# andreeaiana/newsreclib

Measured on AMD Instinct MI355X. Metric: impressions/sec (train step) NRMS MINDsmall-shape, higher is better.
Workload: dtype f32 (projections: 3xbf16 split MFMA); 1 GPU; NRMS pretrained-emb (d=300, 15 heads, Q=200) MINDsmall-shaped train step: B=128/GPU, H=50, C=5, L=30, V=70000, dropout 0.2, Adam lr 1e-4 (BASELINE.json configs[1]); global_batch=128, parallelism=dp1, gemm_engine=bf16x3

## Files before the change

### include/newsreclib_amd.h

```cpp
#ifndef NEWSRECLIB_AMD_H
#define NEWSRECLIB_AMD_H

#include <stddef.h>
#include <stdint.h>

#ifdef __cplusplus
extern "C" {
#endif

#define NRL_ABI_VERSION 19

#define NRL_OK 0
#define NRL_E_INVALID (-1)
#define NRL_E_WORKSPACE (-2)
#define NRL_E_HIP (-3)

typedef struct NrlBlockParams {
  const float* in_proj_weight;
  const float* in_proj_bias;
  const float* out_proj_weight;
  const float* out_proj_bias;
  const float* att_weight;
  const float* att_bias;
  const float* att_query;
// ... 26 lines not shown
int32_t nrl_get_options(void);

int nrl_prof_enable(int32_t on);
int nrl_prof_read(double* total_ms, int64_t* launches, double* total_flops);

uint32_t nrl_dropout_key(uint64_t seed, uint32_t stream);
int nrl_dropout_mask(uint8_t* keep, int64_t n_elems, double p, uint64_t seed, uint32_t stream,
                     void* stream_handle);

size_t nrl_sort_positions_workspace_bytes(int64_t n, int64_t vocab);
int nrl_sort_positions(const int64_t* ids, int64_t n, int64_t vocab, int64_t* order, void* ws, size_t ws_bytes,
                       void* stream);

size_t nrl_news_encoder_workspace_bytes(int64_t n_news, int32_t seq_len, int32_t embed_dim,
                                        int32_t num_heads, int32_t query_dim);
int nrl_news_encoder_fwd(const NrlBlockParams* p, const float* emb_table, int64_t vocab,
                         const int64_t* ids, int64_t n_news, int32_t seq_len, double p_drop,
                         uint64_t seed, uint32_t stream0, int32_t save_for_backward, float* out,
                         void* ws, size_t ws_bytes, void* stream);
int32_t nrl_token_table_supported(int32_t seq_len, int32_t embed_dim, int32_t num_heads, int32_t query_dim);
size_t nrl_token_table_bytes(int64_t vocab, int32_t embed_dim, int32_t num_heads, int32_t query_dim);
int nrl_token_table_build(const NrlBlockParams* p, const float* emb_table, int64_t vocab, void* table, size_t table_bytes,
                          void* stream);
size_t nrl_news_encoder_fwd_table_workspace_bytes(int64_t n_news, int32_t seq_len, int32_t num_heads);
int nrl_news_encoder_fwd_table(const NrlBlockParams* p, const void* table, size_t table_bytes, int64_t vocab,
                               const int64_t* ids, int64_t n_news, int32_t seq_len, float* out, void* ws, size_t ws_bytes,
                               void* stream);
int nrl_news_encoder_bwd(const NrlBlockParams* p, const NrlBlockGrads* g, const float* emb_table,
                         float* d_emb_table, int64_t vocab, const int64_t* ids, const int64_t* sorted_positions,
                         int64_t n_news, int32_t seq_len, double p_drop, uint64_t seed,
// ... 192 lines not shown
                            void* ws, size_t ws_bytes, int32_t image_ready, void* stream);
int nrl_linear_dgrad_gelu_img(const float* w, const float* d_c, const float* pre, int64_t m, int32_t n, int32_t k, float* d_pre,
                              void* ws, size_t ws_bytes, int32_t image_ready, void* stream);
int32_t nrl_linear_gelu_supported(int32_t n_wide);
int32_t nrl_linear3_supported(int32_t n, int32_t k);
size_t nrl_linear3_workspace_bytes(int32_t n, int32_t k);
int nrl_linear3_fwd_img(const float* a, const float* w0, const float* w1, const float* w2, const float* b0, const float* b1,
                        const float* b2, int64_t m, int32_t n, int32_t k, float* c, void* ws, size_t ws_bytes, int32_t image_ready,
                        void* stream);
int nrl_linear3_dgrad_img(const float* d_c, const float* w0, const float* w1, const float* w2, int64_t m, int32_t n, int32_t k,
                          const float* add, float* d_a, void* ws, size_t ws_bytes, int32_t image_ready, void* stream);
int nrl_linear_dgrad_add_img(const float* d_c, const float* w, int64_t m, int32_t n, int32_t k, const float* add, float* d_a,
                             void* ws, size_t ws_bytes, int32_t image_ready, void* stream);
int nrl_embedding_grad(const float* d_out, const int64_t* ids, const int64_t* sorted_positions, int64_t n_ids, int32_t dim,
                       int64_t padding_idx, float* d_table, void* stream);
size_t nrl_linear_workspace_bytes(int32_t n, int32_t k);
int nrl_linear_fwd(const float* a, const float* w, const float* bias, int64_t m, int32_t n,
                   int32_t k, float* c, void* ws, size_t ws_bytes, void* stream);
int nrl_linear_bwd(const float* a, const float* w, const float* d_c, int64_t m, int32_t n, int32_t k, float* d_a,
                   float* d_w, float* d_bias, void* ws, size_t ws_bytes, void* stream);
int nrl_linear_fwd_img(const float* a, const float* w, const float* bias, int64_t m, int32_t n, int32_t k,
                       float* c, void* ws, size_t ws_bytes, int32_t image_ready, void* stream);
int nrl_linear_bwd_img(const float* a, const float* w, const float* d_c, int64_t m, int32_t n, int32_t k, float* d_a,
                       float* d_w, float* d_bias, void* ws, size_t ws_bytes, int32_t image_ready, void* stream);

int32_t nrl_sdpa_supported(int64_t n_batch, int32_t seq_len, int32_t num_heads, int32_t head_dim);
int nrl_sdpa_fwd(const float* q, const float* k, const float* v, const uint8_t* key_keep, int64_t n_batch, int32_t seq_len,
                 int32_t num_heads, int32_t head_dim, float scale, double p_drop, uint64_t seed, uint32_t stream0, float* out,
                 float* lse, void* stream);
int nrl_sdpa_bwd(const float* q, const float* k, const float* v, const uint8_t* key_keep, const float* out, const float* d_out,
// ... 252 lines not shown
```

### newsreclib_amd/_lib.py

```python
from __future__ import annotations

import ctypes
import os
from ctypes import POINTER, c_char_p, c_double, c_float, c_int32, c_int64, c_size_t, c_uint8, c_uint32, c_uint64, c_void_p

_PKG = os.path.dirname(os.path.abspath(__file__))
LIB_PATH = os.path.join(_PKG, "libnewsreclib_amd.so")
ABI_VERSION = 19


class NrlBlockParams(ctypes.Structure):
    _fields_ = [
        ("in_proj_weight", c_void_p), ("in_proj_bias", c_void_p),
        ("out_proj_weight", c_void_p), ("out_proj_bias", c_void_p),
        ("att_weight", c_void_p), ("att_bias", c_void_p), ("att_query", c_void_p),
        ("embed_dim", c_int32), ("num_heads", c_int32), ("query_dim", c_int32), ("gemm_engine", c_int32),
        ("options", c_int32),
    ]


OPTIONS_EXPLICIT = 0x40000000


class NrlBlockGrads(ctypes.Structure):
# ... 87 lines not shown
SIGNATURES = {
    "nrl_abi_version": (c_int32, []),
    "nrl_build_id": (c_char_p, []),
    "nrl_last_error": (c_char_p, []),
    "nrl_set_gemm_engine": (c_int32, [c_int32]),
    "nrl_get_gemm_engine": (c_int32, []),
    "nrl_set_option": (c_int32, [c_char_p, c_int32]),
    "nrl_get_options": (c_int32, []),
    "nrl_prof_enable": (c_int32, [c_int32]),
    "nrl_prof_read": (c_int32, [POINTER(c_double), POINTER(c_int64), POINTER(c_double)]),
    "nrl_dropout_key": (c_uint32, [c_uint64, c_uint32]),
    "nrl_dropout_mask": (c_int32, [c_void_p, c_int64, c_double, c_uint64, c_uint32, c_void_p]),
    "nrl_sort_positions_workspace_bytes": (c_size_t, [c_int64, c_int64]),
    "nrl_sort_positions": (c_int32, [c_void_p, c_int64, c_int64, c_void_p, c_void_p, c_size_t, c_void_p]),
    "nrl_news_encoder_workspace_bytes": (c_size_t, [c_int64, c_int32, c_int32, c_int32, c_int32]),
    "nrl_news_encoder_fwd": (c_int32, [POINTER(NrlBlockParams), c_void_p, c_int64, c_void_p, c_int64, c_int32,
                                       c_double, c_uint64, c_uint32, c_int32, c_void_p, c_void_p, c_size_t,
                                       c_void_p]),
    "nrl_token_table_supported": (c_int32, [c_int32, c_int32, c_int32, c_int32]),
    "nrl_token_table_bytes": (c_size_t, [c_int64, c_int32, c_int32, c_int32]),
    "nrl_token_table_build": (c_int32, [POINTER(NrlBlockParams), c_void_p, c_int64, c_void_p, c_size_t, c_void_p]),
    "nrl_news_encoder_fwd_table_workspace_bytes": (c_size_t, [c_int64, c_int32, c_int32]),
    "nrl_news_encoder_fwd_table": (c_int32, [POINTER(NrlBlockParams), c_void_p, c_size_t, c_int64, c_void_p, c_int64, c_int32,
                                             c_void_p, c_void_p, c_size_t, c_void_p]),
    "nrl_news_encoder_bwd": (c_int32, [POINTER(NrlBlockParams), POINTER(NrlBlockGrads), c_void_p, c_void_p, c_int64,
                                       c_void_p, c_void_p, c_int64, c_int32, c_double, c_uint64, c_uint32,
                                       c_void_p, c_int32, c_void_p, c_size_t, c_void_p]),
    "nrl_user_encoder_workspace_bytes": (c_size_t, [c_int64, c_int64, c_int32, c_int32, c_int32]),
    "nrl_user_encoder_fwd": (c_int32, [POINTER(NrlBlockParams), c_void_p, c_int64, c_int64, c_double, c_uint64,
                                       c_uint32, c_int32, c_int32, c_void_p, c_void_p, c_size_t, c_void_p]),
# ... 189 lines not shown
                                     c_size_t, c_int32, c_void_p]),
    "nrl_linear_gelu_fwd_img": (c_int32, [c_void_p, c_void_p, c_void_p, c_int64, c_int32, c_int32, c_void_p, c_void_p, c_void_p,
                                          c_size_t, c_int32, c_void_p]),
    "nrl_linear_dgrad_gelu_img": (c_int32, [c_void_p, c_void_p, c_void_p, c_int64, c_int32, c_int32, c_void_p, c_void_p, c_size_t,
                                            c_int32, c_void_p]),
    "nrl_linear_gelu_supported": (c_int32, [c_int32]),
    "nrl_linear3_supported": (c_int32, [c_int32, c_int32]),
    "nrl_linear3_workspace_bytes": (c_size_t, [c_int32, c_int32]),
    "nrl_linear3_fwd_img": (c_int32, [c_void_p, c_void_p, c_void_p, c_void_p, c_void_p, c_void_p, c_void_p, c_int64, c_int32, c_int32,
                                      c_void_p, c_void_p, c_size_t, c_int32, c_void_p]),
    "nrl_linear3_dgrad_img": (c_int32, [c_void_p, c_void_p, c_void_p, c_void_p, c_int64, c_int32, c_int32, c_void_p, c_void_p,
                                        c_void_p, c_size_t, c_int32, c_void_p]),
    "nrl_linear_dgrad_add_img": (c_int32, [c_void_p, c_void_p, c_int64, c_int32, c_int32, c_void_p, c_void_p, c_void_p, c_size_t,
                                           c_int32, c_void_p]),
    "nrl_embedding_grad": (c_int32, [c_void_p, c_void_p, c_void_p, c_int64, c_int32, c_int64, c_void_p, c_void_p]),
    "nrl_linear_bwd_img": (c_int32, [c_void_p, c_void_p, c_void_p, c_int64, c_int32, c_int32, c_void_p, c_void_p, c_void_p,
                                     c_void_p, c_size_t, c_int32, c_void_p]),
}

_lib = None


def load() -> ctypes.CDLL:
    global _lib
    if _lib is not None:
        return _lib
    import torch
    if not os.path.exists(LIB_PATH):
        raise RuntimeError(
            f"{LIB_PATH} is missing: the HIP extension was not built (run `python -m newsreclib_amd._build` "
# ... 22 lines not shown


def set_gemm_engine(name: str) -> None:
    if name not in ENGINES:
        raise ValueError(f"unknown GEMM engine {name!r}; choose from {sorted(ENGINES)}")
    check(load().nrl_set_gemm_engine(ENGINES[name]), "nrl_set_gemm_engine")


def get_gemm_engine() -> str:
    code = load().nrl_get_gemm_engine()
    return {v: k for k, v in ENGINES.items()}[code]


OPTION_NAMES = ("news_fused", "news_fused_bwd", "news_attn_mfma", "news_planes", "news_od_planes", "news_aa_planes",
                "wgrad_2step", "wgrad_ws", "rowpanel", "x3_dma", "news_tail", "news_tail_bwd", "user_fork", "news_fork",
                "news_qkv_planes", "news_pad_share", "news_tail_od", "user_proj")


def set_option(name: str, value: bool) -> None:
    check(load().nrl_set_option(name.encode(), int(bool(value))), "nrl_set_option")


def options_mask() -> int:
    return int(load().nrl_get_options())


def options_word() -> int:
    return OPTIONS_EXPLICIT | options_mask()


def require_options(mask: int, what: str) -> None:
# ... 20 lines not shown
```

### newsreclib_amd/csrc/nrl_api.hip

```cpp
#include "nrl_api_internal.h"

namespace nrl {

static thread_local char g_err[512] = "";

void set_error(const char* fmt, ...) {
  va_list ap;
  va_start(ap, fmt);
  vsnprintf(g_err, sizeof(g_err), fmt, ap);
  va_end(ap);
}

ProfState g_prof;
std::atomic<int> g_default_engine{ENGINE_BF16X3};
thread_local int t_engine = -1;
thread_local int64_t t_opts = -1;

static const char* const kOptName[O_COUNT] = {"news_fused", "news_fused_bwd", "news_attn_mfma", "news_planes", "news_od_planes",
                                              "news_aa_planes", "wgrad_2step", "wgrad_ws", "rowpanel", "x3_dma", "news_tail",
                                              "news_tail_bwd", "user_fork", "news_fork", "news_qkv_planes", "news_pad_share", "news_tail_od", "user_proj"};
static const char* const kOptEnv[O_COUNT] = {"NRL_NEWS_FUSED", "NRL_NEWS_FUSED_BWD", "NRL_NEWS_ATTN_MFMA", "NRL_NEWS_PLANES",
                                             "NRL_NEWS_OD_PLANES", "NRL_NEWS_AA_PLANES", "NRL_WGRAD_2STEP", "NRL_WGRAD_WS",
                                             "NRL_ROWPANEL", "NRL_X3_DMA", "NRL_NEWS_TAIL", "NRL_NEWS_TAIL_BWD", "NRL_USER_FORK",
                                             "NRL_NEWS_FORK", "NRL_NEWS_QKV_PLANES", "NRL_NEWS_PAD_SHARE", "NRL_NEWS_TAIL_OD", "NRL_USER_PROJ"};
std::atomic<uint32_t> g_opt_default{[] {
  uint32_t m = 0;
  for (int i = 0; i < O_COUNT; ++i) {
    const bool dflt = i != O_NEWS_FUSED_BWD && i != O_USER_FORK && i != O_NEWS_TAIL_OD;
    const char* e = getenv(kOptEnv[i]);
    bool v = e == nullptr ? dflt : (dflt ? e[0] != '0' : e[0] == '1');
    if (opt_retired(i)) v = false;
    m |= v ? (1u << i) : 0u;
  }
  return m;
}()};

struct ForkSet {
  hipStream_t s[2] = {nullptr, nullptr};
  hipEvent_t fork = nullptr, join[2] = {nullptr, nullptr};
};
static int fork_set(ForkSet** out) {
  thread_local ForkSet sets[64];
  int dev = 0;
  NRL_HIP(hipGetDevice(&dev));
  ForkSet& f = sets[dev & 63];
  if (f.fork == nullptr) {
    for (int i = 0; i < 2; ++i) {
      NRL_HIP(hipStreamCreateWithFlags(&f.s[i], hipStreamNonBlocking));
      NRL_HIP(hipEventCreateWithFlags(&f.join[i], hipEventDisableTiming));
    }
    NRL_HIP(hipEventCreateWithFlags(&f.fork, hipEventDisableTiming));
  }
  *out = &f;
  return NRL_OK;
}

constexpr int LIN_PANEL_BLOCKS = 16;
static inline int lin_panels(int n_out) { return (n_out + 16 * LIN_PANEL_BLOCKS - 1) / (16 * LIN_PANEL_BLOCKS); }
static inline size_t lin_image_elems(int n_out, int k_red) {
  return (size_t)lin_panels(n_out) * rp_image_elems(LIN_PANEL_BLOCKS, rp_kblocks(k_red, false));
}
static inline bool lin_panels_on(int n_out) { return opt(O_ROWPANEL) && n_out >= 16 * LIN_PANEL_BLOCKS; }
template <class Epi>
static int linear_panels(const float* a, const float* src, int64_t sn, int64_t sk, int n_out, int k_red, const Epi& epi,
                         int64_t m, uint16_t* img, hipStream_t st, bool build = true) {
// ... 53 lines not shown
}
int nrl_get_gemm_engine(void) { return g_default_engine.load(); }

int nrl_set_option(const char* name, int32_t value) {
  NRL_REQUIRE(name != nullptr, "set_option: null name");
  for (int i = 0; i < O_COUNT; ++i)
    if (!strcmp(name, kOptName[i])) {
      NRL_REQUIRE(value == 0 || !opt_retired(i), "set_option: '%s' was retired in ABI v14 (its kernel lost its A/B and lives in "
                  "tools/experimental/; the bit is reserved and must stay 0)", name);
      if (value != 0) g_opt_default.fetch_or(1u << i);
      else g_opt_default.fetch_and(~(1u << i));
      return NRL_OK;
    }
  set_error("set_option: unknown option '%s' (news_fused, news_fused_bwd, news_attn_mfma, news_planes, news_od_planes, "
            "news_aa_planes, wgrad_2step, wgrad_ws, rowpanel, x3_dma, news_tail, news_tail_bwd, user_fork, news_fork, news_qkv_planes, "
            "news_pad_share, news_tail_od, user_proj)", name);
  return NRL_E_INVALID;
}

int32_t nrl_get_options(void) { return (int32_t)g_opt_default.load(); }

uint32_t nrl_dropout_key(uint64_t seed, uint32_t stream) { return dropout_key(seed, stream); }

int nrl_dropout_mask(uint8_t* keep, int64_t n_elems, double p, uint64_t seed, uint32_t stream,
                     void* stream_handle) {
  NRL_REQUIRE(keep != nullptr && n_elems >= 0 && p >= 0.0 && p < 1.0, "dropout_mask: bad arguments");
  return dropout_mask(keep, n_elems, make_dropout(p, seed, stream), (hipStream_t)stream_handle);
}

size_t nrl_news_encoder_workspace_bytes(int64_t n_news, int32_t seq_len, int32_t embed_dim,
                                        int32_t num_heads, int32_t query_dim) {
// ... 210 lines not shown
  NRL_TRY(block_planes(p, s, w, false, &bp, st, slabs ? s.heads : 0));
  sb_.forked = news_fork_on(sb_);
  SideFork side;
  hipEvent_t side_in_join = nullptr;
  if (phase != 2) {
    if (sb_.forked) {
      ForkSet* fs = nullptr;
      NRL_TRY(fork_set(&fs));
      side.s = fs->s[0]; side.fork = fs->fork; side.join = fs->join[0];
    }
    NRL_TRY(block_bwd_phase1(p, g, sb_, w, bp, d2, d_out, st, slabs, sb_.forked ? &side : nullptr));
    if (slabs) {
      NewsAttnBwdArgs a;
      a.qkv_hm = w.qkv; a.d_o = w.d_o; a.lse = w.lse; a.dqkv = w.dqkv; a.n_news = n_news; a.L = seq_len; a.D = s.D;
      a.heads = s.heads; a.scale = s.geom.scale; a.hpw = 1; a.planes = planes ? 1 : 0;
      if (planes && opt(O_NEWS_QKV_PLANES)) NRL_TRY(launch_news_attn_bwd_p(a, st));
      else NRL_TRY(launch_news_attn_bwd(a, st));
      if (news_fork_in_on(sb_, planes)) {
        ForkSet* fs = nullptr;
        NRL_TRY(fork_set(&fs));
        const int si = news_fork_in_mode() == 2 ? 0 : 1;
        NRL_HIP(hipEventRecord(fs->fork, st));
        NRL_HIP(hipStreamWaitEvent(fs->s[si], fs->fork, 0));
        NRL_TRY(block_wgrad_in_planes(g, w.x, sb_, w, fs->s[si]));
        NRL_HIP(hipEventRecord(fs->join[1], fs->s[si]));
        side_in_join = fs->join[1];
      }
    }
    const KCSlab dq_hp{w.dqkv, s.M};
    const KCPlanes dq_pl{reinterpret_cast<const unsigned char*>(w.dqkv), s.pad_rows};
    if (sorted_positions != nullptr) {
      float* dx = w.d_o;
      const EpiLinear epi{dx, s.D, nullptr, 0, d1, s.D};
// ... 9 lines not shown
        if (planes) NRL_TRY(rp_dispatch(dq_pl, bp.rp.in_d_hp, EpiNewsRows<EpiLinear>{epi, seq_len}, s.pad_rows, s.D, s.heads * 64, st));
        else if (slabs) NRL_TRY(rp_dispatch(dq_hp, bp.rp.in_d_hp, epi, s.M, s.D, s.heads * 64, st));
        else NRL_TRY(gemm_dgrad(w.dqkv, p->in_proj_weight, bp.in, epi, s.M, 3 * s.D, s.D, st, bp.rp.on ? &bp.rp.in_d : nullptr));
        NRL_TRY(embedding_grad_sorted(dx, ids, sorted_positions, s.M, s.D, d_emb_table, st));
      }
    } else {
      const EpiScatter epi{d_emb_table, ids, s.D, d1};
      if (planes) NRL_TRY(rp_dispatch(dq_pl, bp.rp.in_d_hp, EpiNewsRows<EpiScatter>{epi, seq_len}, s.pad_rows, s.D, s.heads * 64, st));
      else if (slabs) NRL_TRY(rp_dispatch(dq_hp, bp.rp.in_d_hp, epi, s.M, s.D, s.heads * 64, st));
      else NRL_TRY(gemm_dgrad(w.dqkv, p->in_proj_weight, bp.in, epi, s.M, 3 * s.D, s.D, st, bp.rp.on ? &bp.rp.in_d : nullptr));
    }
  }
  if (phase != 2 && sb_.forked) NRL_HIP(hipStreamWaitEvent(st, side.join, 0));
  if (side_in_join != nullptr) NRL_HIP(hipStreamWaitEvent(st, side_in_join, 0));
  if (phase != 1) NRL_TRY(block_bwd_phase2(g, w.x, sb_, w, st, slabs, planes));
  return NRL_OK;
}

size_t nrl_user_encoder_workspace_bytes(int64_t batch, int64_t hist_len, int32_t embed_dim,
                                        int32_t num_heads, int32_t query_dim) {
  return block_ws_floats(batch * hist_len, embed_dim, query_dim, num_heads, true) * sizeof(float);
}

int nrl_user_encoder_fwd(const NrlBlockParams* p, const float* hist, int64_t batch, int64_t hist_len,
                         double p_drop, uint64_t seed, uint32_t stream0, int32_t input_dropout,
                         int32_t save_for_backward, float* out, void* ws, size_t ws_bytes, void* stream) {
  NRL_TRY(check_params(p));
  const EngineScope engine_scope(p->gemm_engine);
  const OptScope opt_scope(p->options);
  NRL_REQUIRE(hist && out && batch > 0 && hist_len > 0, "user_encoder_fwd: bad arguments");
// ... 231 lines not shown
  return launch_rp_gemm<LIN_PANEL_BLOCKS, 4, 0, 2>(A, im, EpiStore{d_a, k}, m, k, 3 * n, st, P);
}

int nrl_linear_dgrad_add_img(const float* d_c, const float* w, int64_t m, int32_t n, int32_t k, const float* add, float* d_a,
                             void* ws, size_t ws_bytes, int32_t image_ready, void* stream) {
  NRL_REQUIRE(d_c && w && add && d_a && m >= 0 && n > 0 && k > 0 && k % 4 == 0 && n % 4 == 0, "linear_dgrad_add: bad arguments");
  NRL_REQUIRE((((uintptr_t)d_c | (uintptr_t)w | (uintptr_t)add | (uintptr_t)d_a) & 15) == 0, "linear_dgrad_add: 16-byte alignment");
  NRL_REQUIRE(cur_engine() == ENGINE_BF16X3 && lin_panels_on(k), "linear_dgrad_add: bf16x3 engine and k >= 256 (nrl_linear_gelu_supported)");
  NRL_REQUIRE(ws != nullptr && ((uintptr_t)ws & 255) == 0 && ws_bytes >= nrl_linear_workspace_bytes(n, k), "linear_dgrad_add: workspace");
  if (m == 0) return NRL_OK;
  return linear_panels(d_c, w, 1, k, k, n, EpiAddStore{d_a, k, add}, m, (uint16_t*)ws, (hipStream_t)stream, image_ready == 0);
}

int32_t nrl_linear_gelu_supported(int32_t n_wide) { return (cur_engine() == ENGINE_BF16X3 && lin_panels_on(n_wide)) ? 1 : 0; }

int nrl_embedding_grad(const float* d_out, const int64_t* ids, const int64_t* sorted_positions, int64_t n_ids, int32_t dim,
                       int64_t padding_idx, float* d_table, void* stream) {
  NRL_REQUIRE(d_out && ids && sorted_positions && d_table && n_ids >= 0 && dim > 0, "embedding_grad: bad arguments");
  return embedding_grad_any(d_out, ids, sorted_positions, n_ids, dim, padding_idx, d_table, (hipStream_t)stream);
}

size_t nrl_linear_workspace_bytes(int32_t n, int32_t k) {
  size_t e = split_weight_elems(n, k);
  if (lin_image_elems(n, k) > e) e = lin_image_elems(n, k);
  if (lin_image_elems(k, n) > e) e = lin_image_elems(k, n);
  return align_up(e * sizeof(uint16_t), 256);
}

int nrl_linear_fwd(const float* a, const float* w, const float* bias, int64_t m, int32_t n, int32_t k,
                   float* c, void* ws, size_t ws_bytes, void* stream) {
// ... 61 lines not shown
```

### newsreclib_amd/csrc/nrl_api_internal.h

```cpp
#pragma once
#include <stdarg.h>
#include <stdlib.h>
#include <string.h>

#include <atomic>
#include <utility>
#include <vector>

#include "nrl_gemm.h"
#include "nrl_gemm_bf16x3.h"
#include "nrl_gemm_bf16x3_dma.h"
#include "nrl_rowpanel.h"
#include "nrl_gemm_ws.h"
#include "nrl_news_fused.h"
#include "nrl_news_tail_api.h"
#include "nrl_user_tail.h"
#include "nrl_wgrad_planes.h"
#include "nrl_kernels.h"
#include "nrl_conv.h"
#include "nrl_gru_fused.h"

namespace nrl {

struct ProfState {
// ... 41 lines not shown

enum { ENGINE_F32 = 0, ENGINE_BF16X3 = 1 };
extern std::atomic<int> g_default_engine;
extern thread_local int t_engine;
static inline int cur_engine() { return t_engine >= 0 ? t_engine : g_default_engine.load(std::memory_order_relaxed); }
struct EngineScope {
  int prev;
  explicit EngineScope(int per_call) : prev(t_engine) {
    t_engine = per_call > 0 ? per_call - 1 : g_default_engine.load(std::memory_order_relaxed);
  }
  ~EngineScope() { t_engine = prev; }
};
static inline bool engine_field_ok(int v) { return v >= 0 && v <= 2; }
enum {
  O_NEWS_FUSED = 0, O_NEWS_FUSED_BWD, O_NEWS_ATTN_MFMA, O_NEWS_PLANES, O_NEWS_OD_PLANES, O_NEWS_AA_PLANES, O_WGRAD_2STEP,
  O_WGRAD_WS, O_ROWPANEL, O_X3_DMA, O_NEWS_TAIL, O_NEWS_TAIL_BWD, O_USER_FORK, O_NEWS_FORK, O_NEWS_QKV_PLANES, O_NEWS_PAD_SHARE, O_NEWS_TAIL_OD, O_USER_PROJ, O_COUNT
};
static inline bool opt_retired(int bit) { return bit == O_NEWS_FUSED_BWD || bit == O_NEWS_TAIL_OD; }
extern std::atomic<uint32_t> g_opt_default;
extern thread_local int64_t t_opts;
static inline bool opt(int bit) {
  const uint32_t m = t_opts >= 0 ? (uint32_t)t_opts : g_opt_default.load(std::memory_order_relaxed);
  return (m >> bit) & 1u;
}
struct OptScope {
  int64_t prev;
  explicit OptScope(int32_t per_call) : prev(t_opts) {
    t_opts = (per_call & NRL_OPTIONS_EXPLICIT) ? (int64_t)(per_call & ((1 << O_COUNT) - 1))
                                               : (int64_t)g_opt_default.load(std::memory_order_relaxed);
  }
  ~OptScope() { t_opts = prev; }
// ... 538 lines not shown
  }
  if (!attention_elsewhere) {
    if (block_attn_x3(s)) NRL_TRY(attn_bwd_x3(w.qkv, w.o, w.d_o, w.lse, w.dqkv, s.geom, st));
    else NRL_TRY(attn_bwd(w.qkv, w.o, w.d_o, w.lse, w.dqkv, s.geom, st));
  }
  return NRL_OK;
}

static inline int news_fork_in_mode() {
  static const int v = [] { const char* e = getenv("NRL_NEWS_FORK_IN"); return e != nullptr ? atoi(e) : 2; }();
  return v;
}
static inline bool news_fork_in_on(const BlockShape& s, bool bf16_planes) {
  return news_fork_in_mode() != 0 && bf16_planes && news_fork_on(s) && s.forked;
}
static int block_wgrad_in_planes(const NrlBlockGrads* G, const float* x_rows, const BlockShape& s, const BlockWs& w, hipStream_t st) {
  const int D = s.D;
  const size_t scratch_avail = opt(O_WGRAD_2STEP) ? qkv_elems(s.M, s.D, s.heads, s.pad_rows) : 0;
  static const int wp_splits = [] { const char* e = getenv("NRL_WGRAD_PLANES_SPLITS"); return e ? atoi(e) : 32; }();
  const EpiAtomicWBHeads epi_w{G->in_proj_weight, D, G->in_proj_bias, D, s.heads, s.dh};
  float* const sc_w = wgrad_planes_scratch_floats(s.heads, 20, wp_splits) <= scratch_avail ? w.qkv : nullptr;
  if (wgrad_planes_waves() == 4) return launch_wgrad_planes<0, 4>(w.dqkv, x_rows, s.pool_groups, s.heads, 20, D + 1, epi_w, wp_splits, st, sc_w);
  return launch_wgrad_planes<0, 8>(w.dqkv, x_rows, s.pool_groups, s.heads, 20, D + 1, epi_w, wp_splits, st, sc_w);
}

static int block_bwd_phase2(const NrlBlockGrads* G, const float* x_rows, const BlockShape& s, const BlockWs& w,
                            hipStream_t st, bool dqkv_head_planes = false, bool bf16_planes = false) {
  const int D = s.D, Q = s.Q;
  const size_t scratch_avail = (bf16_planes && opt(O_WGRAD_2STEP)) ? qkv_elems(s.M, s.D, s.heads, s.pad_rows) : 0;
  auto scratch_for = [&](size_t need) -> float* { return need <= scratch_avail ? w.qkv : nullptr; };
  float* const sc = opt(O_WGRAD_2STEP) && !dqkv_head_planes && !bf16_planes ? w.qkv : nullptr;
  const size_t sc_n = sc != nullptr ? qkv_elems(s.M, s.D, s.heads, s.pad_rows) : 0;
  const bool forked = news_fork_on(s) && s.forked;
  if (!forked && s.aa_planes && s.od_planes) {
    NRL_TRY(block_wgrads_back_half(G, s, w, st, w.qkv, scratch_avail));
  } else if (!forked) {
    if (s.aa_planes) {
      static const int sp = [] { const char* e = getenv("NRL_WGRAD_PLANES_AA_SPLITS"); return e ? atoi(e) : 128; }();
// ... 84 lines not shown
```

### newsreclib_amd/csrc/nrl_gemm.h

```cpp
#pragma once
#include <type_traits>

#include "nrl_common.h"

namespace nrl {

using f32x4 = __attribute__((ext_vector_type(4))) float;

constexpr int GEMM_BK = 16;
enum { SRC_KC = 0, SRC_RC = 1 };

__device__ __forceinline__ float4 f4zero() { return make_float4(0.f, 0.f, 0.f, 0.f); }

__device__ __forceinline__ void store4_stream(float* p, const float4& v) {
  typedef float nt_f32x4 __attribute__((ext_vector_type(4)));
  __builtin_nontemporal_store(nt_f32x4{v.x, v.y, v.z, v.w}, reinterpret_cast<nt_f32x4*>(p));
}
__device__ __forceinline__ void store4(float* p, const float4& v, int stream) {
  if (stream) store4_stream(p, v);
  else *reinterpret_cast<float4*>(p) = v;
}


__device__ const float nrl_dma_zero16[4] = {0.f, 0.f, 0.f, 0.f};
// ... 550 lines not shown
    if (cb < heads) { head = cb; d = c; }
    else { head = 4 * (cb - heads) + (c >> 2); d = 16 + (c & 3); }
    if (head < heads)
      atomicAdd(r.out + head * 20 + d, v);
    else if (head == heads && d == 16 && db != nullptr)
      atomicAdd(db + r.m, v);
  }
};

struct EpiAtomicWBHeads {
  float* dw;
  int64_t ldc;
  float* db;
  int n_w;
  int heads, dh;
  struct Row {
    float* out;
    int64_t m;
  };
  __device__ __forceinline__ Row row(int64_t m) const {
    const int head = (int)(m >> 6), c = (int)(m & 63);
    if (head >= heads || c >= 3 * dh) return Row{nullptr, 0};
    const int part = c / dh, d = c - part * dh;
    const int64_t r = (int64_t)part * heads * dh + head * dh + d;
    return Row{dw + r * ldc, r};
  }
  __device__ __forceinline__ void operator()(const Row& r, int64_t, int n, float v) const {
    if (r.out == nullptr) return;
    if (n < n_w)
      atomicAdd(r.out + n, v);
    else if (n == n_w && db != nullptr)
      atomicAdd(db + r.m, v);
  }
};

struct EpiScatter {
// ... 422 lines not shown
```

### newsreclib_amd/csrc/nrl_kernels.hip

```cpp
#include <math.h>
#include <stdlib.h>

#include "nrl_kernels.h"
#include <cfloat>

namespace nrl {

template <int DH>
__device__ __forceinline__ float dot_row(const float (&q)[DH], const float* row) {
  const float4* r4 = reinterpret_cast<const float4*>(row);
  float acc = 0.f;
#pragma unroll
  for (int d4 = 0; d4 < DH / 4; ++d4) {
    const float4 kv = r4[d4];
    acc = fmaf(q[4 * d4 + 0], kv.x, acc);
    acc = fmaf(q[4 * d4 + 1], kv.y, acc);
    acc = fmaf(q[4 * d4 + 2], kv.z, acc);
    acc = fmaf(q[4 * d4 + 3], kv.w, acc);
  }
  return acc;
}

template <int DH>
__device__ __forceinline__ void axpy_row(float a, const float* row, float (&o)[DH]) {
// ... 1138 lines not shown
          }
          cur = id;
          acc0 = acc1 = 0.f;
        }
        acc0 += r0[u];
        acc1 += r1[u];
      }
    }
  }
  if (cur > 0) {
    if (d0) atomicAdd(d_table + cur * D + tid, acc0);
    if (d1) atomicAdd(d_table + cur * D + tid + 256, acc1);
  }
}

int embedding_grad_sorted(const float* dx, const int64_t* ids, const int64_t* order, int64_t n_rows, int D,
                          float* d_table, hipStream_t stream, const int32_t* cidx) {
  if (n_rows == 0) return NRL_OK;
  NRL_REQUIRE(D <= 512, "embedding_grad_sorted: dim > 512 unsupported");
  hipLaunchKernelGGL(embedding_grad_sorted_kernel, dim3((unsigned)ceil_div(n_rows, EMB_SEG_ROWS)), dim3(256), 0,
                     stream, dx, ids, order, n_rows, D, d_table, cidx);
  NRL_LAUNCH_CHECK();
  return NRL_OK;
}

__global__ void __launch_bounds__(256)
    embedding_grad_any_kernel(const float* __restrict__ dx, const int64_t* __restrict__ ids, const int64_t* __restrict__ order,
                              int64_t n_rows, int D, int64_t padding_idx, float* __restrict__ d_table) {
  __shared__ int64_t s_pos[EMB_SEG_ROWS], s_id[EMB_SEG_ROWS];
  const int64_t beg = (int64_t)blockIdx.x * EMB_SEG_ROWS;
  const int64_t end = beg + EMB_SEG_ROWS < n_rows ? beg + EMB_SEG_ROWS : n_rows;
  const int n = (int)(end - beg);
  const int tid = threadIdx.x;
  if (tid < EMB_SEG_ROWS) {
// ... 314 lines not shown
```

### newsreclib_amd/csrc/nrl_news_fused.h

```cpp
#pragma once
#include <type_traits>

#include "nrl_rowpanel.h"

namespace nrl {

constexpr int NF_WAVES = 8;
constexpr int NF_KB = 10;
constexpr int NF_IMG_LD = 68;
constexpr int NF_IMG_FLOATS = 32 * NF_IMG_LD;
constexpr int NF_RING = 5 * 16384;

struct NewsFusedArgs {
  const float* table;
  const int64_t* ids;
  const uint16_t* img;
  int64_t n_news;
  int L, D, heads, dh;
  float scale;
  Dropout drop1;
  float* o;
  unsigned char* o_planes;
  float* x_save;
  unsigned char* x_planes;
// ... 758 lines not shown
  NRL_LAUNCH_CHECK();
  return NRL_OK;
}


struct NewsAttnBwdArgs {
  const float* qkv_hm;
  const float* d_o;
  const float* lse;
  float* dqkv;
  int64_t n_news;
  int L, D, heads;
  float scale;
  int hpw;
  int planes;
};

constexpr int NAB_WAVES = 4;
constexpr int NAB_DO_FLOATS = 32 * 20;
constexpr int NAB_VEC_FLOATS = 64;
constexpr int NAB_WAVE_FLOATS = NF_IMG_FLOATS + NAB_DO_FLOATS + NAB_VEC_FLOATS;

template <int DH, int OCC, int ABL = 0>
__global__ void __launch_bounds__(NAB_WAVES * 64, OCC) news_attn_bwd_kernel(const NewsAttnBwdArgs P) {
  static_assert(DH == 20, "image packing assumes dh = 20");
  __shared__ __attribute__((aligned(16))) float smem[NAB_WAVES * NAB_WAVE_FLOATS];
  const int tid = threadIdx.x;
  const int lane = tid & 63;
  const int wave = __builtin_amdgcn_readfirstlane(tid >> 6);
  const int l15 = lane & 15, g = lane >> 4;
// ... 295 lines not shown

template <int DH, int OCC, int ABL = 0>
__global__ void __launch_bounds__(NAB_WAVES * 64, OCC) news_attn_bwd_p_kernel(const NewsAttnBwdArgs P) {
  static_assert(DH == 20, "plane rows hold 20 features");
  __shared__ __attribute__((aligned(16))) unsigned char smem[NAB_WAVES * NAP_WAVE_BYTES];
  const int tid = threadIdx.x;
  const int lane = tid & 63;
  const int wave = __builtin_amdgcn_readfirstlane(tid >> 6);
  const int l15 = lane & 15, g = lane >> 4;
  unsigned char* const in = smem + wave * NAP_WAVE_BYTES;
  float* const image = reinterpret_cast<float*>(in);
  float* const vec = reinterpret_cast<float*>(in + NAP_IN);
  const uint32_t in_lds = (uint32_t)(uintptr_t)(__attribute__((address_space(3))) unsigned char*)smem + (uint32_t)wave * NAP_WAVE_BYTES;

  const int L = P.L, D = P.D, heads = P.heads, hpw = P.hpw;
  const int groups = heads / hpw;
  const int64_t unit = (int64_t)blockIdx.x * NAB_WAVES + wave;
  const int64_t news = unit / groups;
  if (news >= P.n_news) return;
  const int h0 = (int)(unit - news * groups) * hpw;
  const int64_t row0 = news * L;
  const float* const do_base = P.d_o + row0 * (int64_t)D;

  auto get_head_inputs = [&](int hd, f32x4 (&qv)[8], float4 (&dv)[3], float& ls) __attribute__((always_inline)) {
    int ln = lane;
    asm volatile("" : "+v"(ln));
    const float* slab = P.qkv_hm + (news * heads + hd) * (int64_t)L * 64;
#pragma unroll
    for (int pass = 0; pass < 8; ++pass) {
      const int slot_i = pass * 64 + ln;
      const bool ok = (slot_i >> 4) < L;
      qv[pass] = *reinterpret_cast<const f32x4*>(slab + (ok ? 4 * slot_i : 0));
      if (!ok) qv[pass] = f32x4{0.f, 0.f, 0.f, 0.f};
    }
#pragma unroll
// ... 255 lines not shown
#pragma unroll
      for (int pass = 0; pass < 4; ++pass) {
        const int ch = pass * 64 + ln;
        float* dst = out + (ch >> 5) * 256 + (ch & 31) * 4;
        store4(dst, stv[2 * pass], !(ABL & 8));
        store4(dst + 128, stv[2 * pass + 1], !(ABL & 8));
      }
    } else {
#pragma unroll
      for (int pass = 0; pass < 8; ++pass)
        asm volatile("" ::"v"(stv[pass].x), "v"(stv[pass].y), "v"(stv[pass].z), "v"(stv[pass].w));
    }
  }
}

template <int OCC = 2, int ABL = 0>
static inline int launch_news_attn_bwd_p(const NewsAttnBwdArgs& a_in, hipStream_t st) {
  if (a_in.n_news <= 0) return NRL_OK;
  NRL_REQUIRE(a_in.planes == 1, "news_attn_bwd_p: dqkv goes out as fragment-block planes");
  NewsAttnBwdArgs a = a_in;
  a.hpw = a.heads % 5 == 0 ? 5 : (a.heads % 3 == 0 ? 3 : 1);
  const int64_t units = a.n_news * (a.heads / a.hpw);
  const int64_t blocks = ceil_div(units, NAB_WAVES);
  NRL_REQUIRE(blocks < (1LL << 31), "news grid too large");
  hipLaunchKernelGGL((news_attn_bwd_p_kernel<20, OCC, ABL>), dim3((unsigned)blocks), dim3(NAB_WAVES * 64), 0, st, a);
  NRL_LAUNCH_CHECK();
  return NRL_OK;
}



}
```

Before: 46350 impressions/s.

## Pipeline news attention backward by head groups with overlapped in-proj wgrad; vectorize embedding grad

Splits the planes-based news attention backward into per-head-group launches. Each finished group's rows are handed to a side stream that runs the in-projection weight gradient for those heads, so the wgrad overlaps the remaining attention backward. Separately, it adds a float4-vectorized sorted embedding-gradient kernel that merges rows per wave before the atomics, plus new API entry points for the compacted embedding grad and the dqkv workspace offset. The grouped path is gated behind a new option and a specific fork mode, and it adds launches and events per step.

```diff
diff --git a/include/newsreclib_amd.h b/include/newsreclib_amd.h
--- a/include/newsreclib_amd.h
+++ b/include/newsreclib_amd.h
@@ -64,6 +64,8 @@
 
 size_t nrl_news_encoder_workspace_bytes(int64_t n_news, int32_t seq_len, int32_t embed_dim,
                                         int32_t num_heads, int32_t query_dim);
+int nrl_news_encoder_ws_dqkv(int64_t n_news, int32_t seq_len, int32_t embed_dim, int32_t num_heads, int32_t query_dim,
+                             size_t* offset_bytes, size_t* n_bytes);
 int nrl_news_encoder_fwd(const NrlBlockParams* p, const float* emb_table, int64_t vocab,
                          const int64_t* ids, int64_t n_news, int32_t seq_len, double p_drop,
                          uint64_t seed, uint32_t stream0, int32_t save_for_backward, float* out,
@@ -286,6 +288,8 @@
                              void* ws, size_t ws_bytes, int32_t image_ready, void* stream);
 int nrl_embedding_grad(const float* d_out, const int64_t* ids, const int64_t* sorted_positions, int64_t n_ids, int32_t dim,
                        int64_t padding_idx, float* d_table, void* stream);
+int nrl_embedding_grad_sorted(const float* d_rows, const int64_t* ids, const int64_t* sorted_positions, int64_t n_ids, int32_t dim,
+                              int32_t compact, float* d_table, int32_t* scratch, size_t scratch_ints, void* stream);
 size_t nrl_linear_workspace_bytes(int32_t n, int32_t k);
 int nrl_linear_fwd(const float* a, const float* w, const float* bias, int64_t m, int32_t n,
                    int32_t k, float* c, void* ws, size_t ws_bytes, void* stream);
diff --git a/newsreclib_amd/_lib.py b/newsreclib_amd/_lib.py
--- a/newsreclib_amd/_lib.py
+++ b/newsreclib_amd/_lib.py
@@ -125,6 +125,7 @@
     "nrl_sort_positions_workspace_bytes": (c_size_t, [c_int64, c_int64]),
     "nrl_sort_positions": (c_int32, [c_void_p, c_int64, c_int64, c_void_p, c_void_p, c_size_t, c_void_p]),
     "nrl_news_encoder_workspace_bytes": (c_size_t, [c_int64, c_int32, c_int32, c_int32, c_int32]),
+    "nrl_news_encoder_ws_dqkv": (c_int32, [c_int64, c_int32, c_int32, c_int32, c_int32, c_void_p, c_void_p]),
     "nrl_news_encoder_fwd": (c_int32, [POINTER(NrlBlockParams), c_void_p, c_int64, c_void_p, c_int64, c_int32,
                                        c_double, c_uint64, c_uint32, c_int32, c_void_p, c_void_p, c_size_t,
                                        c_void_p]),
@@ -344,6 +345,8 @@
     "nrl_linear_dgrad_add_img": (c_int32, [c_void_p, c_void_p, c_int64, c_int32, c_int32, c_void_p, c_void_p, c_void_p, c_size_t,
                                            c_int32, c_void_p]),
     "nrl_embedding_grad": (c_int32, [c_void_p, c_void_p, c_void_p, c_int64, c_int32, c_int64, c_void_p, c_void_p]),
+    "nrl_embedding_grad_sorted": (c_int32, [c_void_p, c_void_p, c_void_p, c_int64, c_int32, c_int32, c_void_p, c_void_p, c_size_t,
+                                            c_void_p]),
     "nrl_linear_bwd_img": (c_int32, [c_void_p, c_void_p, c_void_p, c_int64, c_int32, c_int32, c_void_p, c_void_p, c_void_p,
                                      c_void_p, c_size_t, c_int32, c_void_p]),
 }
@@ -396,7 +399,7 @@
 
 OPTION_NAMES = ("news_fused", "news_fused_bwd", "news_attn_mfma", "news_planes", "news_od_planes", "news_aa_planes",
                 "wgrad_2step", "wgrad_ws", "rowpanel", "x3_dma", "news_tail", "news_tail_bwd", "user_fork", "news_fork",
-                "news_qkv_planes", "news_pad_share", "news_tail_od", "user_proj")
+                "news_qkv_planes", "news_pad_share", "news_tail_od", "user_proj", "news_bwd_groups")
 
 
 def set_option(name: str, value: bool) -> None:
diff --git a/newsreclib_amd/csrc/nrl_api.hip b/newsreclib_amd/csrc/nrl_api.hip
--- a/newsreclib_amd/csrc/nrl_api.hip
+++ b/newsreclib_amd/csrc/nrl_api.hip
@@ -18,11 +18,13 @@
 
 static const char* const kOptName[O_COUNT] = {"news_fused", "news_fused_bwd", "news_attn_mfma", "news_planes", "news_od_planes",
                                               "news_aa_planes", "wgrad_2step", "wgrad_ws", "rowpanel", "x3_dma", "news_tail",
-                                              "news_tail_bwd", "user_fork", "news_fork", "news_qkv_planes", "news_pad_share", "news_tail_od", "user_proj"};
+                                              "news_tail_bwd", "user_fork", "news_fork", "news_qkv_planes", "news_pad_share", "news_tail_od", "user_proj",
+                                              "news_bwd_groups"};
 static const char* const kOptEnv[O_COUNT] = {"NRL_NEWS_FUSED", "NRL_NEWS_FUSED_BWD", "NRL_NEWS_ATTN_MFMA", "NRL_NEWS_PLANES",
                                              "NRL_NEWS_OD_PLANES", "NRL_NEWS_AA_PLANES", "NRL_WGRAD_2STEP", "NRL_WGRAD_WS",
                                              "NRL_ROWPANEL", "NRL_X3_DMA", "NRL_NEWS_TAIL", "NRL_NEWS_TAIL_BWD", "NRL_USER_FORK",
-                                             "NRL_NEWS_FORK", "NRL_NEWS_QKV_PLANES", "NRL_NEWS_PAD_SHARE", "NRL_NEWS_TAIL_OD", "NRL_USER_PROJ"};
+                                             "NRL_NEWS_FORK", "NRL_NEWS_QKV_PLANES", "NRL_NEWS_PAD_SHARE", "NRL_NEWS_TAIL_OD", "NRL_USER_PROJ",
+                                             "NRL_NEWS_BWD_GROUPS"};
 std::atomic<uint32_t> g_opt_default{[] {
   uint32_t m = 0;
   for (int i = 0; i < O_COUNT; ++i) {
@@ -35,9 +37,11 @@
   return m;
 }()};
 
+constexpr int FORK_GROUPS = 4;
 struct ForkSet {
   hipStream_t s[2] = {nullptr, nullptr};
   hipEvent_t fork = nullptr, join[2] = {nullptr, nullptr};
+  hipEvent_t grp[FORK_GROUPS] = {nullptr, nullptr, nullptr, nullptr};
 };
 static int fork_set(ForkSet** out) {
   thread_local ForkSet sets[64];
@@ -49,6 +53,7 @@
       NRL_HIP(hipStreamCreateWithFlags(&f.s[i], hipStreamNonBlocking));
       NRL_HIP(hipEventCreateWithFlags(&f.join[i], hipEventDisableTiming));
     }
+    for (int i = 0; i < FORK_GROUPS; ++i) NRL_HIP(hipEventCreateWithFlags(&f.grp[i], hipEventDisableTiming));
     NRL_HIP(hipEventCreateWithFlags(&f.fork, hipEventDisableTiming));
   }
   *out = &f;
@@ -132,7 +137,7 @@
     }
   set_error("set_option: unknown option '%s' (news_fused, news_fused_bwd, news_attn_mfma, news_planes, news_od_planes, "
             "news_aa_planes, wgrad_2step, wgrad_ws, rowpanel, x3_dma, news_tail, news_tail_bwd, user_fork, news_fork, news_qkv_planes, "
-            "news_pad_share, news_tail_od, user_proj)", name);
+            "news_pad_share, news_tail_od, user_proj, news_bwd_groups)", name);
   return NRL_E_INVALID;
 }
 
@@ -373,9 +378,29 @@
       NewsAttnBwdArgs a;
       a.qkv_hm = w.qkv; a.d_o = w.d_o; a.lse = w.lse; a.dqkv = w.dqkv; a.n_news = n_news; a.L = seq_len; a.D = s.D;
       a.heads = s.heads; a.scale = s.geom.scale; a.hpw = 1; a.planes = planes ? 1 : 0;
-      if (planes && opt(O_NEWS_QKV_PLANES)) NRL_TRY(launch_news_attn_bwd_p(a, st));
+      const int hpw = news_attn_bwd_hpw(s.heads), n_groups = s.heads / hpw;
+      const bool grouped = planes && opt(O_NEWS_QKV_PLANES) && opt(O_NEWS_BWD_GROUPS) && news_fork_in_on(sb_, planes) &&
+                           news_fork_in_mode() == 2 && n_groups >= 2 && n_groups <= FORK_GROUPS;
+      if (grouped) {
+        ForkSet* fs = nullptr;
+        NRL_TRY(fork_set(&fs));
+        int issued = 0;
+        for (int gi = 0; gi < n_groups; ++gi) {
+          a.h_first = gi * hpw; a.h_count = hpw;
+          NRL_TRY(launch_news_attn_bwd_p(a, st));
+          const int ready = gi + 1 == n_groups ? s.heads : (gi + 1) * hpw / 4 * 4;
+          if (ready > issued) {
+            NRL_HIP(hipEventRecord(fs->grp[gi], st));
+            NRL_HIP(hipStreamWaitEvent(fs->s[0], fs->grp[gi], 0));
+            NRL_TRY(block_wgrad_in_planes(g, w.x, sb_, w, fs->s[0], issued, ready - issued, w.t, (size_t)s.M * s.Q));
+            issued = ready;
+          }
+        }
+        NRL_HIP(hipEventRecord(fs->join[1], fs->s[0]));
+        side_in_join = fs->join[1];
+      } else if (planes && opt(O_NEWS_QKV_PLANES)) NRL_TRY(launch_news_attn_bwd_p(a, st));
       else NRL_TRY(launch_news_attn_bwd(a, st));
-      if (news_fork_in_on(sb_, planes)) {
+      if (!grouped && news_fork_in_on(sb_, planes)) {
         ForkSet* fs = nullptr;
         NRL_TRY(fork_set(&fs));
         const int si = news_fork_in_mode() == 2 ? 0 : 1;
@@ -415,6 +440,19 @@
   if (phase != 2 && sb_.forked) NRL_HIP(hipStreamWaitEvent(st, side.join, 0));
   if (side_in_join != nullptr) NRL_HIP(hipStreamWaitEvent(st, side_in_join, 0));
   if (phase != 1) NRL_TRY(block_bwd_phase2(g, w.x, sb_, w, st, slabs, planes));
+  return NRL_OK;
+}
+
+int nrl_news_encoder_ws_dqkv(int64_t n_news, int32_t seq_len, int32_t embed_dim, int32_t num_heads, int32_t query_dim,
+                             size_t* offset_bytes, size_t* n_bytes) {
+  NRL_REQUIRE(offset_bytes && n_bytes && n_news > 0 && seq_len > 0 && embed_dim > 0 && num_heads > 0 && query_dim > 0,
+              "news_encoder_ws_dqkv: bad arguments");
+  BlockShape s{};
+  s.M = n_news * seq_len; s.D = embed_dim; s.Q = query_dim; s.heads = num_heads;
+  s.pad_rows = news_pad_rows(n_news, seq_len, embed_dim, num_heads);
+  const size_t x = align_up(x_elems(s.M, s.D, s.pad_rows), 64), q = qkv_elems(s.M, s.D, s.heads, s.pad_rows);
+  *offset_bytes = (x + align_up(q, 64)) * sizeof(float);
+  *n_bytes = q * sizeof(float);
   return NRL_OK;
 }
 
@@ -676,6 +714,16 @@
 
 int32_t nrl_linear_gelu_supported(int32_t n_wide) { return (cur_engine() == ENGINE_BF16X3 && lin_panels_on(n_wide)) ? 1 : 0; }
 
+int nrl_embedding_grad_sorted(const float* d_rows, const int64_t* ids, const int64_t* sorted_positions, int64_t n_ids, int32_t dim,
+                              int32_t compact, float* d_table, int32_t* scratch, size_t scratch_ints, void* stream) {
+  NRL_REQUIRE(d_rows && ids && sorted_positions && d_table && n_ids >= 0 && dim > 0, "embedding_grad_sorted: bad arguments");
+  if (compact == 0) return embedding_grad_sorted(d_rows, ids, sorted_positions, n_ids, dim, d_table, (hipStream_t)stream);
+  NRL_REQUIRE(scratch != nullptr && scratch_ints >= live_compact_ints(n_ids), "embedding_grad_sorted: scratch of 2 n + n / 2048 + 9 int32");
+  const int32_t *list = nullptr, *cidx = nullptr, *n_live = nullptr;
+  NRL_TRY(live_compact(ids, n_ids, scratch, &list, &cidx, &n_live, (hipStream_t)stream));
+  return embedding_grad_sorted(d_rows, ids, sorted_positions, n_ids, dim, d_table, (hipStream_t)stream, cidx);
+}
+
 int nrl_embedding_grad(const float* d_out, const int64_t* ids, const int64_t* sorted_positions, int64_t n_ids, int32_t dim,
                        int64_t padding_idx, float* d_table, void* stream) {
   NRL_REQUIRE(d_out && ids && sorted_positions && d_table && n_ids >= 0 && dim > 0, "embedding_grad: bad arguments");
diff --git a/newsreclib_amd/csrc/nrl_api_internal.h b/newsreclib_amd/csrc/nrl_api_internal.h
--- a/newsreclib_amd/csrc/nrl_api_internal.h
+++ b/newsreclib_amd/csrc/nrl_api_internal.h
@@ -79,7 +79,7 @@
 static inline bool engine_field_ok(int v) { return v >= 0 && v <= 2; }
 enum {
   O_NEWS_FUSED = 0, O_NEWS_FUSED_BWD, O_NEWS_ATTN_MFMA, O_NEWS_PLANES, O_NEWS_OD_PLANES, O_NEWS_AA_PLANES, O_WGRAD_2STEP,
-  O_WGRAD_WS, O_ROWPANEL, O_X3_DMA, O_NEWS_TAIL, O_NEWS_TAIL_BWD, O_USER_FORK, O_NEWS_FORK, O_NEWS_QKV_PLANES, O_NEWS_PAD_SHARE, O_NEWS_TAIL_OD, O_USER_PROJ, O_COUNT
+  O_WGRAD_WS, O_ROWPANEL, O_X3_DMA, O_NEWS_TAIL, O_NEWS_TAIL_BWD, O_USER_FORK, O_NEWS_FORK, O_NEWS_QKV_PLANES, O_NEWS_PAD_SHARE, O_NEWS_TAIL_OD, O_USER_PROJ, O_NEWS_BWD_GROUPS, O_COUNT
 };
 static inline bool opt_retired(int bit) { return bit == O_NEWS_FUSED_BWD || bit == O_NEWS_TAIL_OD; }
 extern std::atomic<uint32_t> g_opt_default;
@@ -648,14 +648,25 @@
 static inline bool news_fork_in_on(const BlockShape& s, bool bf16_planes) {
   return news_fork_in_mode() != 0 && bf16_planes && news_fork_on(s) && s.forked;
 }
-static int block_wgrad_in_planes(const NrlBlockGrads* G, const float* x_rows, const BlockShape& s, const BlockWs& w, hipStream_t st) {
+static int block_wgrad_in_planes(const NrlBlockGrads* G, const float* x_rows, const BlockShape& s, const BlockWs& w, hipStream_t st,
+                                 int head0 = 0, int n_heads = 0, float* scratch = nullptr, size_t scratch_floats = 0) {
   const int D = s.D;
-  const size_t scratch_avail = opt(O_WGRAD_2STEP) ? qkv_elems(s.M, s.D, s.heads, s.pad_rows) : 0;
-  static const int wp_splits = [] { const char* e = getenv("NRL_WGRAD_PLANES_SPLITS"); return e ? atoi(e) : 32; }();
-  const EpiAtomicWBHeads epi_w{G->in_proj_weight, D, G->in_proj_bias, D, s.heads, s.dh};
-  float* const sc_w = wgrad_planes_scratch_floats(s.heads, 20, wp_splits) <= scratch_avail ? w.qkv : nullptr;
-  if (wgrad_planes_waves() == 4) return launch_wgrad_planes<0, 4>(w.dqkv, x_rows, s.pool_groups, s.heads, 20, D + 1, epi_w, wp_splits, st, sc_w);
-  return launch_wgrad_planes<0, 8>(w.dqkv, x_rows, s.pool_groups, s.heads, 20, D + 1, epi_w, wp_splits, st, sc_w);
+  static const int wp_splits0 = [] { const char* e = getenv("NRL_WGRAD_PLANES_SPLITS"); return e ? atoi(e) : 32; }();
+  int wp_splits = wp_splits0;
+  const void* dqkv = w.dqkv;
+  if (n_heads > 0) {
+    NRL_REQUIRE(head0 % 4 == 0 && head0 + n_heads <= s.heads, "wgrad_in_planes: a head range starts at a row tile");
+    wp_splits = wp_splits0 * ((s.heads + 3) / 4) / ((n_heads + 3) / 4);
+    dqkv = reinterpret_cast<const unsigned char*>(w.dqkv) + (size_t)head0 * (size_t)s.pool_groups * 8192;
+  } else {
+    n_heads = s.heads;
+    scratch = w.qkv;
+    scratch_floats = opt(O_WGRAD_2STEP) ? qkv_elems(s.M, s.D, s.heads, s.pad_rows) : 0;
+  }
+  const EpiAtomicWBHeads epi_w{G->in_proj_weight, D, G->in_proj_bias, D, s.heads, s.dh, head0};
+  float* const sc_w = wgrad_planes_scratch_floats(n_heads, 20, wp_splits) <= scratch_floats ? scratch : nullptr;
+  if (wgrad_planes_waves() == 4) return launch_wgrad_planes<0, 4>(dqkv, x_rows, s.pool_groups, n_heads, 20, D + 1, epi_w, wp_splits, st, sc_w);
+  return launch_wgrad_planes<0, 8>(dqkv, x_rows, s.pool_groups, n_heads, 20, D + 1, epi_w, wp_splits, st, sc_w);
 }
 
 static int block_bwd_phase2(const NrlBlockGrads* G, const float* x_rows, const BlockShape& s, const BlockWs& w,
diff --git a/newsreclib_amd/csrc/nrl_gemm.h b/newsreclib_amd/csrc/nrl_gemm.h
--- a/newsreclib_amd/csrc/nrl_gemm.h
+++ b/newsreclib_amd/csrc/nrl_gemm.h
@@ -588,12 +588,13 @@
   float* db;
   int n_w;
   int heads, dh;
+  int head0 = 0;
   struct Row {
     float* out;
     int64_t m;
   };
   __device__ __forceinline__ Row row(int64_t m) const {
-    const int head = (int)(m >> 6), c = (int)(m & 63);
+    const int head = head0 + (int)(m >> 6), c = (int)(m & 63);
     if (head >= heads || c >= 3 * dh) return Row{nullptr, 0};
     const int part = c / dh, d = c - part * dh;
     const int64_t r = (int64_t)part * heads * dh + head * dh + d;
diff --git a/newsreclib_amd/csrc/nrl_kernels.hip b/newsreclib_amd/csrc/nrl_kernels.hip
--- a/newsreclib_amd/csrc/nrl_kernels.hip
+++ b/newsreclib_amd/csrc/nrl_kernels.hip
@@ -1176,10 +1176,135 @@
   }
 }
 
+constexpr int EGV_WAVES = 8, EGV_ROWS = EMB_SEG_ROWS / EGV_WAVES, EGV_BATCH = 4;
+static_assert(EGV_ROWS % EGV_BATCH == 0, "a wave's rows go in whole batches");
+template <int NV>
+__global__ void __launch_bounds__(EGV_WAVES * 64, 8)
+    embedding_grad_sorted_v4_kernel(const float* __restrict__ dx, const int64_t* __restrict__ ids,
+                                    const int64_t* __restrict__ order, int64_t n_rows, int D,
+                                    float* __restrict__ d_table, const int32_t* __restrict__ cidx) {
+  int64_t skip = 0;
+  const bool compact = cidx != nullptr;
+  if (compact) {
+    skip = order[n_rows];
+    if ((int64_t)blockIdx.x * EMB_SEG_ROWS >= n_rows - skip) return;
+    order += skip;
+    n_rows -= skip;
+  }
+  __shared__ int64_t s_id[EMB_SEG_ROWS], s_row[EMB_SEG_ROWS], s_eid[2 * EGV_WAVES];
+  __shared__ __attribute__((aligned(16))) float s_part[2 * EGV_WAVES][512];
+  const int64_t beg = (int64_t)blockIdx.x * EMB_SEG_ROWS;
+  const int64_t end = beg + EMB_SEG_ROWS < n_rows ? beg + EMB_SEG_ROWS : n_rows;
+  const int n = (int)(end - beg);
+  const int tid = threadIdx.x, lane = tid & 63;
+  const int wave = __builtin_amdgcn_readfirstlane(tid >> 6);
+  if (tid < EMB_SEG_ROWS) {
+    const int64_t pos = order[beg + (tid < n ? tid : n - 1)];
+    s_id[tid] = tid < n ? ids[pos] : 0;
+    s_row[tid] = compact ? (int64_t)cidx[pos] : pos;
+  } else if (tid < EMB_SEG_ROWS + 2 * EGV_WAVES) {
+    s_eid[tid - EMB_SEG_ROWS] = -1;
+  }
+  __syncthreads();
+  if (s_id[n - 1] == 0) return;
+  const int D4 = D >> 2;
+  const float4* const dx4 = reinterpret_cast<const float4*>(dx);
+  bool ok[NV];
+  int lv[NV];
+#pragma unroll
+  for (int v = 0; v < NV; ++v) {
+    ok[v] = lane + 64 * v < D4;
+    lv[v] = ok[v] ? lane + 64 * v : D4 - 1;
+  }
+  float4 acc[NV];
+#pragma unroll
+  for (int v = 0; v < NV; ++v) acc[v] = make_float4(0.f, 0.f, 0.f, 0.f);
+  int64_t cur = -1;
+  bool first = true;
+  auto close = [&](bool last) {
+    if (cur > 0) {
+      if (first || last) {
+        const int e = 2 * wave + (first ? 0 : 1);
+#pragma unroll
+        for (int v = 0; v < NV; ++v)
+          if (ok[v]) *reinterpret_cast<float4*>(&s_part[e][4 * (lane + 64 * v)]) = acc[v];
+        if (lane == 0) s_eid[e] = cur;
+      } else {
+#pragma unroll
+        for (int v = 0; v < NV; ++v)
+          if (ok[v]) {
+            float* p = d_table + cur * D + 4 * (lane + 64 * v);
+            atomicAdd(p, acc[v].x);
+            atomicAdd(p + 1, acc[v].y);
+            atomicAdd(p + 2, acc[v].z);
+            atomicAdd(p + 3, acc[v].w);
+          }
+      }
+    }
+  };
+  const int j0 = wave * EGV_ROWS;
+#pragma unroll
+  for (int b = 0; b < EGV_ROWS; b += EGV_BATCH) {
+    float4 r[EGV_BATCH][NV];
+#pragma unroll
+    for (int u = 0; u < EGV_BATCH; ++u) {
+      const float4* row = dx4 + s_row[j0 + b + u] * D4;
+#pragma unroll
+      for (int v = 0; v < NV; ++v) r[u][v] = row[lv[v]];
+    }
+#pragma unroll
+    for (int u = 0; u < EGV_BATCH; ++u) {
+      if (j0 + b + u < n) {
+        const int64_t id = s_id[j0 + b + u];
+        if (id != cur) {
+          if (cur != -1) {
+            close(false);
+            first = false;
+          }
+          cur = id;
+#pragma unroll
+          for (int v = 0; v < NV; ++v) acc[v] = make_float4(0.f, 0.f, 0.f, 0.f);
+        }
+#pragma unroll
+        for (int v = 0; v < NV; ++v) {
+          acc[v].x += r[u][v].x; acc[v].y += r[u][v].y; acc[v].z += r[u][v].z; acc[v].w += r[u][v].w;
+        }
+      }
+    }
+  }
+  if (cur != -1) close(true);
+  __syncthreads();
+  if (tid < D) {
+    float a = 0.f;
+    int64_t c = -1;
+#pragma unroll
+    for (int e = 0; e < 2 * EGV_WAVES; ++e) {
+      const int64_t id = s_eid[e];
+      if (id > 0) {
+        if (id != c) {
+          if (c > 0) atomicAdd(d_table + c * D + tid, a);
+          c = id;
+          a = 0.f;
+        }
+        a += s_part[e][tid];
+      }
+    }
+    if (c > 0) atomicAdd(d_table + c * D + tid, a);
+  }
+}
+
 int embedding_grad_sorted(const float* dx, const int64_t* ids, const int64_t* order, int64_t n_rows, int D,
                           float* d_table, hipStream_t stream, const int32_t* cidx) {
   if (n_rows == 0) return NRL_OK;
-  NRL_REQUIRE(D <= 512, "embedding_grad_sorted: dim > 512 unsupported");
+  NRL_REQUIRE(D > 0 && D <= 512, "embedding_grad_sorted: dim > 512 unsupported");
+  static const bool vec_env = [] { const char* e = getenv("NRL_EMB_GRAD_VEC"); return !(e != nullptr && e[0] == '0'); }();
+  if (vec_env && D % 4 == 0 && ((uintptr_t)dx & 15) == 0) {
+    const dim3 grid((unsigned)ceil_div(n_rows, EMB_SEG_ROWS)), block(EGV_WAVES * 64);
+    if (D <= 256) hipLaunchKernelGGL(embedding_grad_sorted_v4_kernel<1>, grid, block, 0, stream, dx, ids, order, n_rows, D, d_table, cidx);
+    else hipLaunchKernelGGL(embedding_grad_sorted_v4_kernel<2>, grid, block, 0, stream, dx, ids, order, n_rows, D, d_table, cidx);
+    NRL_LAUNCH_CHECK();
+    return NRL_OK;
+  }
   hipLaunchKernelGGL(embedding_grad_sorted_kernel, dim3((unsigned)ceil_div(n_rows, EMB_SEG_ROWS)), dim3(256), 0,
                      stream, dx, ids, order, n_rows, D, d_table, cidx);
   NRL_LAUNCH_CHECK();
diff --git a/newsreclib_amd/csrc/nrl_news_fused.h b/newsreclib_amd/csrc/nrl_news_fused.h
--- a/newsreclib_amd/csrc/nrl_news_fused.h
+++ b/newsreclib_amd/csrc/nrl_news_fused.h
@@ -796,6 +796,8 @@
   float scale;
   int hpw;
   int planes;
+  int h_first = 0;
+  int h_count = 0;
 };
 
 constexpr int NAB_WAVES = 4;
@@ -1121,11 +1123,11 @@
   const uint32_t in_lds = (uint32_t)(uintptr_t)(__attribute__((address_space(3))) unsigned char*)smem + (uint32_t)wave * NAP_WAVE_BYTES;
 
   const int L = P.L, D = P.D, heads = P.heads, hpw = P.hpw;
-  const int groups = heads / hpw;
+  const int groups = P.h_count / hpw;
   const int64_t unit = (int64_t)blockIdx.x * NAB_WAVES + wave;
   const int64_t news = unit / groups;
   if (news >= P.n_news) return;
-  const int h0 = (int)(unit - news * groups) * hpw;
+  const int h0 = P.h_first + (int)(unit - news * groups) * hpw;
   const int64_t row0 = news * L;
   const float* const do_base = P.d_o + row0 * (int64_t)D;
 
@@ -1411,13 +1413,17 @@
   }
 }
 
+static inline int news_attn_bwd_hpw(int heads) { return heads % 5 == 0 ? 5 : (heads % 3 == 0 ? 3 : 1); }
 template <int OCC = 2, int ABL = 0>
 static inline int launch_news_attn_bwd_p(const NewsAttnBwdArgs& a_in, hipStream_t st) {
   if (a_in.n_news <= 0) return NRL_OK;
   NRL_REQUIRE(a_in.planes == 1, "news_attn_bwd_p: dqkv goes out as fragment-block planes");
   NewsAttnBwdArgs a = a_in;
-  a.hpw = a.heads % 5 == 0 ? 5 : (a.heads % 3 == 0 ? 3 : 1);
-  const int64_t units = a.n_news * (a.heads / a.hpw);
+  a.hpw = news_attn_bwd_hpw(a.heads);
+  if (a.h_count == 0) { a.h_first = 0; a.h_count = a.heads; }
+  NRL_REQUIRE(a.h_first >= 0 && a.h_count > 0 && a.h_first % a.hpw == 0 && a.h_count % a.hpw == 0 && a.h_first + a.h_count <= a.heads,
+              "news_attn_bwd_p: the head range must be whole groups of hpw heads");
+  const int64_t units = a.n_news * (a.h_count / a.hpw);
   const int64_t blocks = ceil_div(units, NAB_WAVES);
   NRL_REQUIRE(blocks < (1LL << 31), "news grid too large");
   hipLaunchKernelGGL((news_attn_bwd_p_kernel<20, OCC, ABL>), dim3((unsigned)blocks), dim3(NAB_WAVES * 64), 0, st, a);
```

Result: slower. 44430 impressions/s (-4.1%).
